# Ji4chenLi/t2v-turbo

Hardware: AMD Instinct MI355X
Metric: UNet denoise steps/sec (16f 320x512 latent) (higher is better)
Workload: dtype bf16; 1 GPU; VideoCrafter2 UNet forward, B=1 per GPU, latent (1,4,16,40,64), ctx (1,77,1024), 4-step LCM timestep table, random-init weights (zero-init tensors re-drawn); parallelism=replicas x1, hip_graph=True, graph_captured=True

## Files before the change

### include/t2v_hip.h

```cpp
#ifndef T2V_HIP_H
#define T2V_HIP_H

#ifdef __cplusplus
extern "C" {
#endif

#define T2V_OK 0
#define T2V_EINVAL (-1)
#define T2V_ESHAPE (-2)
#define T2V_EHIP (-3)

#define T2V_F32 0
#define T2V_BF16 1
#define T2V_F16 2

int t2v_version(void);
int t2v_init(void);
const char* t2v_last_error(void);

#define T2V_GEMM_LINEAR 0
#define T2V_GEMM_CONV3X3 1
#define T2V_GEMM_CONV3X3_S2 2
#define T2V_GEMM_CONV3X3_UP2 3
#define T2V_GEMM_TCONV3 4
// ... 103 lines not shown
                    float* ws, float* stats, void* stream);

int t2v_layernorm(const void* x, int ldx, int M, int C, const float* gamma, const float* beta,
                  float eps, void* out, int ldo, void* stream);

int t2v_softmax_rows(void* s, long long rows, int n, int n_pad, int ld, void* stream);

int t2v_attn_spatial(const void* q, int ldq, const void* k, int ldk, const void* vt, int ld_vt,
                     long long vt_img_stride, void* out, int ldo, int n_img, int seq_q, int seq_kv,
                     int heads, int kv_div, float scale, void* stream);

int t2v_attn_temporal(const void* q, int ldq, const void* k, int ldk, const void* v, int ldv,
                      void* out, int ldo, int n_clips, int frames, int hw, int heads, float scale,
                      float* probs, void* stream);

int t2v_ncfhw_to_tokens(const void* x, int dt, int b, int c, int f, int hw, void* out, int ldo,
                        void* stream);
int t2v_tokens_to_ncfhw(const void* tok, int tok_f32, int ld, int b, int c, int f, int hw,
                        void* out, int dt, void* stream);
int t2v_timestep_embedding(const void* t, int t_is_f32, int n, int dim, int guidance_style,
                           void* out_bf16, void* stream);
int t2v_silu(const void* x, void* out, long long n, void* stream);
int t2v_fill_zero(void* p, long long nbytes, void* stream);
int t2v_cast(const void* x, int dt_in, void* out, int dt_out, long long n, void* stream);
int t2v_lincomb3(const float* x, const float* y, const float* z, const float* ca, const float* cb,
                 const float* cc, int nb, long long inner, float* out, void* stream);
int t2v_lcm_step(const float* x, const void* eps, int eps_dt, const float* noise, float sa_t,
                 float sb_t, float c_skip, float c_out, float sa_p, float sb_p, long long n,
                 float* prev, float* denoised, void* stream);
int t2v_video_to_u8(const void* x, int dt, int B, int T, int H, int W, void* out, void* stream);
// ... 215 lines not shown
```

### t2v-turbo_amd/csrc/linear_pr.hip

```cpp
#include "gelu_poly.h"
#if defined(T2V_HOSTSIM) && !defined(T2V_WT_ON)
#define T2V_WT_ON(bit) 0
template <int WT, class V> inline void t2v_store_out16(void* p, const V& v) { *(V*)p = v; }
template <int WT, class V> inline void t2v_store_out8(void* p, const V& v) { *(V*)p = v; }
#endif
#include <cstdlib>
#include <type_traits>

struct LprParams {
    t2v_gemm_desc d;
    int chunks;
    int chunks_per_y;
    int n_out;
    int debug;
};

#ifdef T2V_LPR_ABLATE
#define LABL(bit) (p.debug & (bit))
#else
#define LABL(bit) false
#endif

#ifdef T2V_LPR_TRACE
#define LPR_STAMP() do { if (tr && ti < 31) { if (lane == 0) tr[ti] = __builtin_amdgcn_s_memtime(); ++ti; } } while (0)
#else
#define LPR_STAMP() do { } while (0)
#endif

namespace {
// ... 1 lines not shown
constexpr int kLprWaves = 8;
#ifndef T2V_LPR_RING
#define T2V_LPR_RING 5
#endif
#ifndef T2V_LPR_STAGGER
#define T2V_LPR_STAGGER 0
#endif
#ifdef T2V_LPR_PACKED_GELU
constexpr bool kLprScalarGelu = false;
#else
constexpr bool kLprScalarGelu = true;
#endif
#ifndef T2V_LPR_AF1
#define T2V_LPR_AF1 1
#endif
constexpr int kLprRing = T2V_LPR_RING;
constexpr bool kLprAf1 = T2V_LPR_AF1 != 0;

template <int I, int N, class F>
__device__ __forceinline__ void lpr_static_for(F&& f) {
    if constexpr (I < N) {
        f(std::integral_constant<int, I>{});
        lpr_static_for<I + 1, N>(f);
    }
}

template <int TB, int KS, int EPI, int PRE>
__global__ __launch_bounds__(kLprWaves * 64) __attribute__((amdgpu_waves_per_eu(2, 2))) void linear_pr_kernel(const LprParams p) {
    constexpr int BM = 32 * TB, K = 16 * KS, D = KS % kLprRing == 0 ? kLprRing : 4;
    constexpr bool GEGLU = EPI == 1, RES = EPI == 2;
    constexpr bool XPF = !RES;
// ... 19 lines not shown
    LPR_STAMP();
    unsigned long long* wg_tr = d.ws ? (unsigned long long*)d.ws + 3 * kLprWaves * 32 + (blockIdx.y * gridDim.x + blockIdx.x) * 4 : nullptr;
    if (wg_tr && tid == 0) { wg_tr[0] = __builtin_amdgcn_s_memtime(); wg_tr[2] = (unsigned)__builtin_amdgcn_s_getreg((15 << 11) | (0 << 6) | 4); wg_tr[3] = (unsigned)__builtin_amdgcn_s_getreg((3 << 11) | (0 << 6) | 20); }
#endif
    const int c_begin = blockIdx.y * p.chunks_per_y, c_end = min(p.chunks, c_begin + p.chunks_per_y);

    const int n_run = c_end - c_begin;
    const bool active = wave < n_run;
    int chunk = c_begin + (active ? wave : 0);

    uint4 rres[RES ? TB : 1][2][2];
    auto load_res_all = [&](int ch) {
        if constexpr (RES) {
            unsigned loff = (unsigned)lane;
            asm volatile("" : "+v"(loff));
            loff = ((loff & 31u) * (unsigned)d.ldr + 16u * (loff >> 5)) * 2u;
#pragma unroll
            for (int i = 0; i < TB; ++i) {
                const int row0 = m0 + 32 * i < d.M ? m0 + 32 * i : m0;
                const char* rp = (const char*)d.residual + ((long long)row0 * d.ldr + ch * 64) * 2 + loff;
#pragma unroll
                for (int b = 0; b < 2; ++b) {
                    rres[i][b][0] = *(const uint4*)(rp + 64 * b);
                    rres[i][b][1] = *(const uint4*)(rp + 64 * b + 16);
                }
            }
        }
    };

    constexpr bool LNIN = PRE == 1, GNIN = PRE == 2;
    if constexpr (PRE == 0) {
        constexpr int CG = K / 64, RG = BM / 8, PIECES = RG * CG, PPW = (PIECES + kLprWaves - 1) / kLprWaves;
        uint4 stage[PPW];
        const bf16_t* a = (const bf16_t*)d.a0;
#pragma unroll
// ... 2 lines not shown
            const int rg = pc / CG, cg = pc - rg * CG;
            const int row = 8 * rg + (lane & 7), c = 8 * cg + (lane >> 3);
            const int gm = m0 + row;
            if (pc < PIECES) stage[j] = *(const uint4*)(a + (long long)min(gm, d.M - 1) * d.lda0 + c * 8);
        }
        if (active) load_res_all(chunk);
        float* sb = (float*)(smem + PANEL_BYTES);
        const int nb = (c_end - c_begin) * 64;
        for (int i = tid; i < nb; i += kLprWaves * 64) sb[i] = d.bias ? d.bias[c_begin * 64 + i] : 0.f;
#pragma unroll
        for (int j = 0; j < PPW; ++j) {
            const int pc = wave + kLprWaves * j;
            const int rg = pc / CG, cg = pc - rg * CG;
            const int row = 8 * rg + (lane & 7), c = 8 * cg + (lane >> 3);
            if (pc < PIECES) *(uint4*)(smem + (c * BM + row) * 16) = m0 + row < d.M ? stage[j] : make_uint4(0u, 0u, 0u, 0u);
        }
    } else {
        constexpr int CG = K / 64, RG = BM / 8, RPW = (RG + kLprWaves - 1) / kLprWaves;
        uint4 stage[RPW][CG];
        const bf16_t* a = (const bf16_t*)d.a0;
#pragma unroll
        for (int jr = 0; jr < RPW; ++jr) {
            const int rg = wave + kLprWaves * jr;
            const int gm = m0 + 8 * rg + (lane & 7);
            const bf16_t* ap = a + (long long)min(gm, d.M - 1) * d.lda0 + (lane >> 3) * 8;
#pragma unroll
            for (int cg = 0; cg < CG; ++cg)
                if (rg < RG) stage[jr][cg] = *(const uint4*)(ap + cg * 64);
        }
        float* sb = (float*)(smem + PANEL_BYTES);
// ... 172 lines not shown
            const char* wb = wcur;
            static_assert(KS / D >= 2, "a first and a last iteration");
            lpr_static_for<0, D>([&](auto u) { kstep(wb, 0, u, F{}, T{}); });
            wb += D * 2048;
#pragma unroll 1
            for (int it = 1; it < KS / D - 1; ++it, wb += D * 2048) lpr_static_for<0, D>([&](auto u) { kstep(wb, it * D, u, F{}, F{}); });
            lpr_static_for<0, D>([&](auto u) { kstep(wb, KS - D, u, T{}, F{}); });
        }
        LPR_STAMP();
        int chunk_e = chunk;
        asm volatile("" : "+s"(chunk_e));
        {
            unsigned ao = a_off;
            asm volatile("" : "+v"(ao));
            const unsigned he = ao >= (unsigned)(BM * 16) ? 1u : 0u, le = (ao >> 4) - he * BM;
            const unsigned g_off = (le * (unsigned)d.ldo + 16u * he) * 2u;
            auto put = [&](const float* v, int row0, int col) {
                if (row0 + (int)le < d.M && !LABL(16)) {
                    char* op = (char*)obase + ((long long)row0 * d.ldo + col) * 2 + g_off;
                    t2v_store_out16<T2V_WT_ON(T2V_WT_LINEAR_PR)>(op, pack8(v));
                    t2v_store_out16<T2V_WT_ON(T2V_WT_LINEAR_PR)>(op + 16, pack8(v + 8));
                }
            };
            if constexpr (GEGLU) {
#pragma unroll
                for (int i = 0; i < TB; ++i) {
                    float v[16];
                    if (LABL(8)) {
#pragma unroll
                        for (int e = 0; e < 16; ++e) v[e] = acc[i][0][e] + acc[i][1][e];
                    } else if (LABL(64) || kLprScalarGelu) {
#pragma unroll
                        for (int e = 0; e < 16; ++e) v[e] = acc[i][0][e] * fast_gelu(acc[i][1][e]);
                    } else {
#pragma unroll
                        for (int e = 0; e < 16; e += 2) {
                            const f32x2_t gg = fast_gelu2((f32x2_t){acc[i][1][e], acc[i][1][e + 1]});
                            const f32x2_t vv = (f32x2_t){acc[i][0][e], acc[i][0][e + 1]} * gg;
                            v[e] = vv[0]; v[e + 1] = vv[1];
                        }
                    }
#ifdef T2V_LPR_TRACE
                    if (chunk < c_begin + kLprWaves) { asm volatile("" :: "v"(v[0]), "v"(v[15])); LPR_STAMP(); }
#endif
                    put(v, m0 + 32 * i, chunk_e * 32);
#ifdef T2V_LPR_TRACE
                    if (chunk < c_begin + kLprWaves) LPR_STAMP();
#endif
                }
            } else {
#pragma unroll
                for (int ib = 0; ib < 2 * TB; ++ib) {
                    const int i = ib >> 1, b = ib & 1;
                    float v[16];
#pragma unroll
                    for (int e = 0; e < 16; ++e) v[e] = acc[i][b][e];
                    put(v, m0 + 32 * i, chunk_e * 64 + 32 * b);
                }
            }
        }
        LPR_STAMP();
#ifdef T2V_LPR_TRACE
        if (!has_next && wg_tr && lane == 0) atomicMax(&wg_tr[1], (unsigned long long)__builtin_amdgcn_s_memtime());
#endif
        if (!has_next) break;
        chunk = nchunk;
        wcur = wnext;
        load_res_all(chunk);

    }
}

template <int TB, int KS, int EPI, int PRE = 0>
int lpr_launch(const LprParams& p, int tiles_m, int ny, hipStream_t s) {
    const int smem = 16 * KS * 32 * TB * 2 + p.chunks_per_y * 64 * 4;
    static bool attr_set = false;
    if (!attr_set) {
        hipFuncSetAttribute((const void*)linear_pr_kernel<TB, KS, EPI, PRE>, hipFuncAttributeMaxDynamicSharedMemorySize, 160 * 1024);
        attr_set = true;
    }
    hipLaunchKernelGGL((linear_pr_kernel<TB, KS, EPI, PRE>), dim3(tiles_m, ny), dim3(kLprWaves * 64), smem, s, p);
    T2V_CHECK_LAUNCH();
    return T2V_OK;
}

}

static int g_lpr_debug = 0, g_lpr_force_ny = 0;
extern "C" int t2v_linear_pr_debug(int bits) { g_lpr_debug = bits; return T2V_OK; }
extern "C" int t2v_linear_pr_force_split(int ny) { g_lpr_force_ny = ny; return T2V_OK; }

static int lpr_prepare(const t2v_gemm_desc* dd, LprParams& p, int& cfg, int& tiles_m, int& ny) {
    cfg = 0;
    T2V_REQUIRE(dd && dd->a0 && dd->w && dd->out, T2V_EINVAL, "t2v_linear_pr: null pointer");
    p.d = *dd;
    const t2v_gemm_desc& d = p.d;
    {
        const int n_out = d.act == T2V_ACT_GEGLU ? d.N / 2 : d.N;
        T2V_REQUIRE(d.lda0 >= d.c0 && (!d.a1 || d.lda1 >= d.c1), T2V_EINVAL, "t2v_linear_pr: lda0 < c0 or lda1 < c1");
        T2V_REQUIRE(d.ldo >= n_out && (!d.residual || d.ldr >= n_out) && (!d.rowvec || d.ld_rowvec >= n_out), T2V_EINVAL,
                    "t2v_linear_pr: ldo / ldr / ld_rowvec smaller than the output row");
    }
    if (d.mode != T2V_GEMM_LINEAR || d.a1 || d.c1 || d.batch > 1 || d.alpha != 1.0f || d.out_f32 || d.split_k > 1 || d.drop_thr || d.ln_out ||
        d.rowstat_out || d.colstat_out || d.lnf_stats || d.lora_t || d.rowvec || (d.act != T2V_ACT_NONE && d.act != T2V_ACT_GEGLU))
        return T2V_OK;
    if (d.c0 != 320 && d.c0 != 640 && d.c0 != 512) return T2V_OK;
    if (d.M <= 0 || d.N <= 0 || d.N % 64 || d.lda0 % 8 || d.ldo % 8) return T2V_OK;
    if ((long long)d.M * d.ldo >= (1ll << 31) || (long long)d.M * d.ldr >= (1ll << 31) || (long long)d.N * d.c0 * 2 >= (1ll << 31)) return T2V_OK;
    if (((uintptr_t)d.a0 | (uintptr_t)d.w | (uintptr_t)d.out) % 16) return T2V_OK;
    if (d.residual && (d.act == T2V_ACT_GEGLU || d.ldr % 8 || (uintptr_t)d.residual % 16 || d.M % 32)) return T2V_OK;
    if (d.bias && (uintptr_t)d.bias % 16) return T2V_OK;
    if (d.ln_in) {
        T2V_REQUIRE(d.ln_gamma && d.ln_beta, T2V_EINVAL, "t2v_linear_pr: ln_in without ln_gamma / ln_beta");
        if (d.residual || ((uintptr_t)d.ln_gamma | (uintptr_t)d.ln_beta) % 16) return T2V_OK;
    }
    const int bm = d.c0 == 320 ? 160 : 96;
    if (d.c0 == 512 && (d.residual || d.gn_coef)) return T2V_OK;
    if (d.gn_coef) {
        T2V_REQUIRE(!d.ln_in && d.gn_rows_per_unit > 0, T2V_EINVAL, "t2v_linear_pr: gn_coef with ln_in, or without gn_rows_per_unit");
        if (d.residual || (uintptr_t)d.gn_coef % 16 || d.gn_rows_per_unit % bm || d.M % d.gn_rows_per_unit) return T2V_OK;
    }
    p.chunks = d.N / 64;
    p.n_out = d.act == T2V_ACT_GEGLU ? d.N / 2 : d.N;
    tiles_m = (d.M + bm - 1) / bm;
    ny = 1;
    if (g_lpr_force_ny > 0) ny = g_lpr_force_ny;
    else if (tiles_m < 256) {
        ny = (256 + tiles_m / 2) / tiles_m;
        const int max_ny = p.chunks / kLprWaves > 0 ? p.chunks / kLprWaves : 1;
        if (ny > max_ny) ny = max_ny;
    }
    if (ny > p.chunks) ny = p.chunks;
    if (ny < 1) ny = 1;
    p.chunks_per_y = (p.chunks + ny - 1) / ny;
    ny = (p.chunks + p.chunks_per_y - 1) / p.chunks_per_y;
    if (d.c0 * bm * 2 + p.chunks_per_y * 256 > 160 * 1024) return T2V_OK;
    p.debug = g_lpr_debug;
    cfg = d.c0 == 320 ? 1 : (d.c0 == 640 ? 2 : 3);
    return T2V_OK;
}

extern "C" int t2v_linear_pr_supported(const t2v_gemm_desc* dd) {
    LprParams p;
    int cfg = 0, tiles_m = 0, ny = 0;
    const int rc = lpr_prepare(dd, p, cfg, tiles_m, ny);
    return rc != T2V_OK ? rc : (cfg > 0 ? 1 : 0);
}

extern "C" int t2v_linear_pr(const t2v_gemm_desc* dd, void* stream) {
    LprParams p;
    int cfg = 0, tiles_m = 0, ny = 0;
// ... 6 lines not shown
        T2V_REQUIRE(epi != 2 && !p.d.gn_coef, T2V_ESHAPE, "t2v_linear_pr: K = 512 takes the plain and the GEGLU epilogue (ask t2v_linear_pr_supported first)");
        if (p.d.ln_in) return epi == 1 ? lpr_launch<3, 32, 1, 1>(p, tiles_m, ny, s) : lpr_launch<3, 32, 0, 1>(p, tiles_m, ny, s);
        return epi == 1 ? lpr_launch<3, 32, 1>(p, tiles_m, ny, s) : lpr_launch<3, 32, 0>(p, tiles_m, ny, s);
    }
    if (p.d.ln_in) {
        if (cfg == 1) return epi == 1 ? lpr_launch<5, 20, 1, 1>(p, tiles_m, ny, s) : lpr_launch<5, 20, 0, 1>(p, tiles_m, ny, s);
        return epi == 1 ? lpr_launch<3, 40, 1, 1>(p, tiles_m, ny, s) : lpr_launch<3, 40, 0, 1>(p, tiles_m, ny, s);
    }
    if (p.d.gn_coef) {
        T2V_REQUIRE(epi == 0, T2V_ESHAPE, "t2v_linear_pr: gn_coef goes with the plain epilogue");
        return cfg == 1 ? lpr_launch<5, 20, 0, 2>(p, tiles_m, ny, s) : lpr_launch<3, 40, 0, 2>(p, tiles_m, ny, s);
    }
    if (cfg == 1) return epi == 1 ? lpr_launch<5, 20, 1>(p, tiles_m, ny, s) : (epi == 2 ? lpr_launch<5, 20, 2>(p, tiles_m, ny, s) : lpr_launch<5, 20, 0>(p, tiles_m, ny, s));
    return epi == 1 ? lpr_launch<3, 40, 1>(p, tiles_m, ny, s) : (epi == 2 ? lpr_launch<3, 40, 2>(p, tiles_m, ny, s) : lpr_launch<3, 40, 0>(p, tiles_m, ny, s));
}
```

### t2v-turbo_amd/csrc/replay.hip

```cpp
#include "common.h"

#include <cstring>
#include <tuple>
#include <type_traits>
#include <utility>

namespace {

template <class T>
inline T slot_as(uint64_t v) {
    if constexpr (std::is_pointer_v<T>) {
        return (T)(uintptr_t)v;
    } else if constexpr (std::is_same_v<T, float>) {
        const uint32_t b = (uint32_t)v;
        float f;
        memcpy(&f, &b, 4);
        return f;
    } else if constexpr (std::is_same_v<T, double>) {
        double d;
        memcpy(&d, &v, 8);
        return d;
    } else {
        return (T)(int64_t)v;
    }
// ... 23 lines not shown
const Entry kTable[] = {
    T2V_ENTRY(t2v_gemm), T2V_ENTRY(t2v_conv_halo), T2V_ENTRY(t2v_linear_pr),
#ifdef T2V_EXPERIMENTAL
    T2V_ENTRY(t2v_ffn_fused),
#endif
    T2V_ENTRY(t2v_conv3x3_small_cin), T2V_ENTRY(t2v_gn_stats),
    T2V_ENTRY(t2v_gn_apply), T2V_ENTRY(t2v_group_norm), T2V_ENTRY(t2v_group_norm_cs), T2V_ENTRY(t2v_gn_stats_cs), T2V_ENTRY(t2v_layernorm),
    T2V_ENTRY(t2v_softmax_rows), T2V_ENTRY(t2v_attn_spatial), T2V_ENTRY(t2v_attn_temporal), T2V_ENTRY(t2v_ncfhw_to_tokens),
    T2V_ENTRY(t2v_tokens_to_ncfhw), T2V_ENTRY(t2v_timestep_embedding), T2V_ENTRY(t2v_silu), T2V_ENTRY(t2v_fill_zero), T2V_ENTRY(t2v_cast),
    T2V_ENTRY(t2v_lincomb3), T2V_ENTRY(t2v_lcm_step), T2V_ENTRY(t2v_gn_bwd), T2V_ENTRY(t2v_softmax_bwd_rows), T2V_ENTRY(t2v_transpose_bf16),
    T2V_ENTRY(t2v_sumpool2x2), T2V_ENTRY(t2v_gn_bwd2), T2V_ENTRY(t2v_layernorm_bwd), T2V_ENTRY(t2v_geglu_fwd), T2V_ENTRY(t2v_geglu_bwd),
    T2V_ENTRY(t2v_scatter2x), T2V_ENTRY(t2v_add_bf16), T2V_ENTRY(t2v_attn_temporal_bwd), T2V_ENTRY(t2v_adamw_step), T2V_ENTRY(t2v_ema_update),
    T2V_ENTRY(t2v_sumsq), T2V_ENTRY(t2v_gather_f32), T2V_ENTRY(t2v_attn_spatial_bwd), T2V_ENTRY(t2v_wgrad_tn), T2V_ENTRY(t2v_wgrad_tn_group),
    T2V_ENTRY(t2v_transpose_pad_bf16), T2V_ENTRY(t2v_dropout_bf16), T2V_ENTRY(t2v_im2col_bf16), T2V_ENTRY(t2v_gn_coef_cs), T2V_ENTRY(t2v_norm_affine_grad),
    T2V_ENTRY(t2v_rowlin_fwd), T2V_ENTRY(t2v_rowlin_bwd_data), T2V_ENTRY(t2v_rowlin_wgrad), T2V_ENTRY(t2v_timestep_embedding_f32), T2V_ENTRY(t2v_dropout_f32),
    T2V_ENTRY(t2v_rank_loss), T2V_ENTRY(t2v_ema_multi),
};
constexpr int kEntries = (int)(sizeof(kTable) / sizeof(kTable[0]));

}

extern "C" int t2v_replay_lookup(const char* name) {
    if (!name) return -1;
    for (int i = 0; i < kEntries; ++i)
        if (strcmp(kTable[i].name, name) == 0) return i;
    return -1;
}


extern "C" int t2v_replay(const unsigned long long* prog, long long nwords, void* stream, int* failed_index) {
    T2V_REQUIRE(prog && nwords >= 0, T2V_EINVAL, "t2v_replay: null program");
// ... 18 lines not shown
```

### t2v-turbo_amd/engine.py

```python
import collections
import os

import torch
import torch.nn as nn

from . import native as nt
from .native import on_tensor_device
from .packs import Packer, effective_weight_bias, is_lora_leaf, leaf_out_channels, params_fingerprint, params_fingerprints
from .unet3d import (Downsample, ResBlock, SpatialTransformer, TemporalTransformer, TimestepEmbedSequential,
                     Upsample)


class BufferPool:

    def __init__(self, device):
        self.device = device
        self.free = collections.defaultdict(list)
        self.live = {}
        self.links = {}
        self.bytes = 0

    def get(self, rows, cols, dtype, zero=False):
        n = rows * cols
        nbytes = ((n * torch.empty((), dtype=dtype).element_size() + 255) // 256) * 256
# ... 158 lines not shown
    linear_pr = os.environ.get("T2V_LINEAR_PR", "1") == "1"
    linear_pr_min_n = {320: int(os.environ.get("T2V_LPR_MIN_N_320", "640")), 640: int(os.environ.get("T2V_LPR_MIN_N_640", "1920")),
                       512: int(os.environ.get("T2V_LPR_MIN_N_512", "1536"))}
    if os.environ.get("T2V_LPR_K512", "1") != "1":
        del linear_pr_min_n[512]

    def _lpr_takes(self, a, w, out, kw):
        if not self.linear_pr or any(k in kw for k in ("ln", "lnf", "colstat", "rowstat")) or not hasattr(self.ops, "linear_pr_supported"):
            return False
        K, N = a.shape[1], kw["N"]
        if K not in self.linear_pr_min_n or w.shape[1] != K or w.shape[0] != N or w.stride(0) != K:
            return False
        if kw.get("act") != nt.ACT_GEGLU and N < self.linear_pr_min_n[K]:
            return False
        return self.ops.linear_pr_supported(a, w, out, **kw) == 1

    ln_in_fill = os.environ.get("T2V_LN_IN", "1") == "1"

    def linear_ln_in(self, a, norm, *, w, bias, act=nt.ACT_NONE):
        if not self.ln_in_fill or tuple(norm.normalized_shape) != (a.shape[1],) or not norm.elementwise_affine:
            return None
        N = w.shape[0]
        out = self.buf(a.shape[0], N // 2 if act == nt.ACT_GEGLU else N)
        kw = dict(M=a.shape[0], N=N, bias=bias, residual=None, act=act,
                  ln_in=(self.pk.f32(norm.weight), self.pk.f32(norm.bias), norm.eps))
        if not self._lpr_takes(a, w, out, kw):
            self.pool.put(out)
            return None
        self.ops.linear_pr(a, self.pk.lpr(w), out, **kw)
        return out
# ... 553 lines not shown
            ops.layernorm(src, pk.f32(norm.weight), pk.f32(norm.bias), norm.eps, ln_buf())
            return box["ln"]

        def foldable(norm, stats):
            return (fold and stats is not None and tuple(norm.normalized_shape) == (C,) and norm.elementwise_affine and
                    C % 64 == 0 and C <= 1280)

        wide = fold and self.fold_ln_wide

        def folded(src, norm, stats, pack, act=nt.ACT_NONE):
            if not foldable(norm, stats):
                return None
            wp, s_vec, t_vec = pack()
            return self.linear(src, None, w=wp, bias=t_vec, act=act, lnf=(stats, norm.eps, s_vec))

        def temporal_attn(attn, norm, src, stats):
            qkv = folded(src, norm, stats if wide else None, lambda: pk.mat_lnf([attn.to_q, attn.to_k, attn.to_v], norm, "qkv_lnf"))
            if qkv is None and src is not box["ln"]:
                qkv = self.linear_ln_in(src, norm, w=pk.cat_mats([attn.to_q, attn.to_k, attn.to_v], "qkv"), bias=None)
            if qkv is None:
                qkv = self.linear(lnorm(norm, src) if src is not box["ln"] else src, None,
                                  w=pk.cat_mats([attn.to_q, attn.to_k, attn.to_v], "qkv"), bias=None)
            o = self.buf(M, inner)
            probs = None
            if attn.record_attn_probs:
                probs = torch.empty(B * hw * attn.heads, F, F, dtype=torch.float32, device=self.device)
                self.plan["probs"].append((attn, probs))
            ops.attn_temporal(qkv[:, :inner], qkv[:, inner:2 * inner], qkv[:, 2 * inner:], o, B, F, hw, attn.heads,
                              attn.scale, probs)
            self.pool.put(qkv)
            return o

        def spatial_self_attn(attn, src):
            qk = self.linear(src, None, w=pk.cat_mats([attn.to_q, attn.to_k], "qk"), bias=None)
            kp = ((hw + 63) // 64) * 64
            vt = self.buf(n_img * inner, kp)
            if kp != hw:
                ops.fill_zero(vt)
            ops.gemm(pk.mat(attn.to_v), src, vt, M=inner, N=hw, batch=n_img, w_strides=(hw * src.stride(0), 0),
                     o_strides=(inner * kp, 0))
            o = self.buf(M, inner)
            ops.attn_spatial(qk[:, :inner], qk[:, inner:], vt, kp, o, n_img, hw, hw, attn.heads, 1, attn.scale)
            self.pool.put(qk, vt)
            return o

        def cross_attn(attn, norm, src, stats):
            q = folded(src, norm, stats, lambda: pk.mat_lnf([attn.to_q], norm, "q_lnf"))
            if q is None:
                q = self.linear(lnorm(norm, src) if src is not box["ln"] else src, attn.to_q, bias=None)
            k, vt, kp, vt_stride = self.context_kv(attn)
            o = self.buf(M, inner)
            ops.attn_spatial(q, k, vt, kp, o, n_img, hw, self.ctx_len, attn.heads, F, attn.scale, vt_stride)
            self.pool.put(q)
            return o

        if temporal:
            o = temporal_attn(a1, blk.norm1, ln1 if ln1 is not None else y, rs)
        else:
            o = spatial_self_attn(a1, ln1 if ln1 is not None else lnorm(blk.norm1, y))
        y1 = self.linear(o, a1.to_out[0], residual=y, ln=(blk.norm2, ln_buf()) if fuse2 else None, want_rs=fold and (wide or not temporal))
        rs1 = self.last_rs
        self.pool.put(o)
        src = box["ln"] if fuse2 else y1
        o = temporal_attn(a2, blk.norm2, src, rs1) if temporal else cross_attn(a2, blk.norm2, src, rs1)
        y2 = self.linear(o, a2.to_out[0], residual=y1, ln=(blk.norm3, ln_buf()) if fuse3 else None, want_rs=wide)
        rs2 = self.last_rs
        self.pool.put(o, y1)
        proj = blk.ff.net[0]
        assert hasattr(proj, "proj"), "non-gated FeedForward is not built by the VideoCrafter2 config"
        if (self.fuse_ff and ops.ffn_fused_supported(C) and tuple(blk.norm3.normalized_shape) == (C,) and blk.norm3.elementwise_affine
                and not fuse3 and leaf_out_channels(blk.ff.net[2]) == C and leaf_out_channels(proj.proj) == 8 * C):
            w1p, b1p, w2p, b2f = pk.ffn(blk.ff, blk.norm3)
            y3 = self.buf(M, C)
            ops.ffn_fused(y2, w1p, b1p, w2p, b2f, blk.norm3.eps, y3)
            self.pool.put(y2, box["ln"])
            return y3
        g = folded(y2, blk.norm3, rs2 if wide else None, lambda: pk.geglu_lnf(proj.proj, blk.norm3), act=nt.ACT_GEGLU)
        if g is None and not fuse3:
            wg, bg = pk.geglu(proj.proj)
            g = self.linear_ln_in(y2, blk.norm3, w=wg, bias=bg, act=nt.ACT_GEGLU)
        if g is None:
            src = box["ln"] if fuse3 else lnorm(blk.norm3, y2)
# ... 69 lines not shown
```

### t2v-turbo_amd/native.py

```python
import ctypes as C
import os

import torch

_PKG = os.path.dirname(os.path.abspath(__file__))
LIB_PATH = os.path.join(_PKG, "libt2v_hip.so")

F32, BF16, F16 = 0, 1, 2
GEMM_LINEAR, GEMM_CONV3X3, GEMM_CONV3X3_S2, GEMM_CONV3X3_UP2, GEMM_TCONV3, GEMM_CONV3X3_S2_PAD01 = range(6)
ACT_NONE, ACT_GEGLU, ACT_SILU = 0, 1, 2

_DT = {torch.float32: F32, torch.bfloat16: BF16, torch.float16: F16}


WGRAD_GROUP_MAX = 8


class WgradProblem(C.Structure):
    _fields_ = [("a", C.c_void_p), ("b", C.c_void_p), ("out", C.c_void_p), ("M", C.c_longlong), ("lda", C.c_int), ("ldb", C.c_int),
                ("ldo", C.c_int), ("R", C.c_int), ("C", C.c_int), ("alpha", C.c_float)]


RANK_LOSS_MAX = 16
RANK_LOSS_WG_LANES = 2048
# ... 188 lines not shown
    "t2v_group_norm_cs_ws_floats": (C.c_longlong, [C.c_int, C.c_int, C.c_int]),
    "t2v_gn_stats_cs": (C.c_int, [C.c_void_p, C.c_int, C.c_void_p, C.c_int, C.c_int, C.c_int, C.c_int, C.c_float, C.c_void_p, C.c_void_p,
                                  C.c_void_p]),
    "t2v_group_norm_cs": (C.c_int, [C.c_void_p, C.c_void_p, C.c_void_p, C.c_int, C.c_int, C.c_void_p, C.c_int, C.c_int, C.c_int, C.c_int,
                                    C.c_int, C.c_float, C.c_void_p, C.c_void_p, C.c_int, C.c_void_p, C.c_void_p, C.c_int, C.c_void_p,
                                    C.c_longlong, C.c_void_p]),
    "t2v_layernorm": (C.c_int, [C.c_void_p, C.c_int, C.c_int, C.c_int, C.c_void_p, C.c_void_p, C.c_float,
                                C.c_void_p, C.c_int, C.c_void_p]),
    "t2v_softmax_rows": (C.c_int, [C.c_void_p, C.c_longlong, C.c_int, C.c_int, C.c_int, C.c_void_p]),
    "t2v_attn_spatial": (C.c_int, [C.c_void_p, C.c_int, C.c_void_p, C.c_int, C.c_void_p, C.c_int, C.c_longlong,
                                   C.c_void_p, C.c_int, C.c_int, C.c_int, C.c_int, C.c_int, C.c_int, C.c_float,
                                   C.c_void_p]),
    "t2v_attn_temporal": (C.c_int, [C.c_void_p, C.c_int, C.c_void_p, C.c_int, C.c_void_p, C.c_int, C.c_void_p,
                                    C.c_int, C.c_int, C.c_int, C.c_int, C.c_int, C.c_float, C.c_void_p,
                                    C.c_void_p]),
    "t2v_ncfhw_to_tokens": (C.c_int, [C.c_void_p, C.c_int, C.c_int, C.c_int, C.c_int, C.c_int, C.c_void_p, C.c_int,
                                      C.c_void_p]),
    "t2v_tokens_to_ncfhw": (C.c_int, [C.c_void_p, C.c_int, C.c_int, C.c_int, C.c_int, C.c_int, C.c_int, C.c_void_p,
                                      C.c_int, C.c_void_p]),
    "t2v_timestep_embedding": (C.c_int, [C.c_void_p, C.c_int, C.c_int, C.c_int, C.c_int, C.c_void_p, C.c_void_p]),
    "t2v_silu": (C.c_int, [C.c_void_p, C.c_void_p, C.c_longlong, C.c_void_p]),
    "t2v_fill_zero": (C.c_int, [C.c_void_p, C.c_longlong, C.c_void_p]),
    "t2v_cast": (C.c_int, [C.c_void_p, C.c_int, C.c_void_p, C.c_int, C.c_longlong, C.c_void_p]),
    "t2v_lincomb3": (C.c_int, [C.c_void_p, C.c_void_p, C.c_void_p, C.c_void_p, C.c_void_p, C.c_void_p, C.c_int,
                               C.c_longlong, C.c_void_p, C.c_void_p]),
    "t2v_gemm_debug": (C.c_int, [C.c_int]),
    "t2v_attn_debug": (C.c_int, [C.c_int]),
    "t2v_gn_coop_enable": (C.c_int, [C.c_int]),
    "t2v_gn_coop_error": (C.c_int, []),
    "t2v_gn_bwd_ws_floats": (C.c_longlong, [C.c_int, C.c_int, C.c_int]),
# ... 68 lines not shown
                                  C.c_float, C.c_void_p, C.c_void_p, C.c_void_p, C.c_longlong, C.c_void_p, C.c_int, C.c_longlong,
                                  C.c_void_p]),
    "t2v_cd_loss_bwd": (C.c_int, [C.c_void_p, C.c_void_p, C.c_void_p, C.c_void_p, C.c_void_p, C.c_int, C.c_int, C.c_longlong, C.c_void_p]),
    "t2v_cd_add_noise": (C.c_int, [C.c_void_p, C.c_void_p, C.c_int, C.c_void_p, C.c_int, C.c_void_p, C.c_void_p, C.c_int, C.c_int,
                                   C.c_longlong, C.c_void_p]),
    "t2v_ddim_reverse_step": (C.c_int, [C.c_void_p, C.c_int, C.c_int, C.c_void_p, C.c_void_p, C.c_int, C.c_void_p, C.c_void_p, C.c_int,
                                        C.c_int, C.c_longlong, C.c_void_p]),
    "t2v_pack_f16_multi": (C.c_int, [C.c_void_p, C.c_int, C.c_void_p, C.c_longlong, C.c_void_p]),
    "t2v_mp_guided_step": (C.c_int, [C.c_void_p, C.c_int, C.c_float, C.c_void_p, C.c_void_p, C.c_void_p, C.c_int, C.c_void_p, C.c_void_p,
                                     C.c_int, C.c_void_p, C.c_int, C.c_void_p, C.c_int, C.c_void_p, C.c_int, C.c_void_p, C.c_int,
                                     C.c_longlong, C.c_void_p]),
    "t2v_video_to_u8": (C.c_int, [C.c_void_p, C.c_int, C.c_int, C.c_int, C.c_int, C.c_int, C.c_void_p, C.c_void_p]),
}
EXPERIMENTAL = ("t2v_gemm2_enable", "t2v_ffn_fused_supported", "t2v_ffn_fused")
EXPORTED = sorted(n for n in _SIGS if n not in EXPERIMENTAL)


def has_experimental(lib=None):
    lib = lib if lib is not None else load()
    return hasattr(lib, "t2v_ffn_fused")


def load(path=None):
    global _lib
    if _lib is not None:
        return _lib
    path = path or os.environ.get("T2V_HIP_LIB", LIB_PATH)
    if not os.path.exists(path):
        raise NativeError(
            f"{path} not found: build it with `python __graft_entry__.py` / "
            f"`python t2v-turbo_amd/csrc/build.py` (hipcc, gfx950). There is no fallback path.")
    try:
        lib = C.CDLL(path)
    except OSError as e:
        raise NativeError(f"cannot load {path}: {e}") from e
    for name, (res, args) in _SIGS.items():
        if name in EXPERIMENTAL and not hasattr(lib, name):
            continue
        fn = getattr(lib, name)
        fn.restype = res
        fn.argtypes = args
    _lib = lib
    return lib


def _check(rc, what):
    if rc != 0:
        msg = _lib.t2v_last_error().decode(errors="replace") if _lib is not None else ""
        raise NativeError(f"{what} failed with code {rc}: {msg}")


def _p(t):
# ... 359 lines not shown
    def layernorm(self, x, gamma, beta, eps, out):
        self._call("t2v_layernorm", _p(x), _row_stride(x), x.shape[0], x.shape[1], _p(gamma), _p(beta), eps, _p(out),
                   _row_stride(out))

    def softmax_rows(self, s, rows, n, n_pad, ld):
        self._call("t2v_softmax_rows", _p(s), rows, n, n_pad, ld)

    def attn_spatial(self, q, k, vt, ld_vt, out, n_img, seq_q, seq_kv, heads, kv_div, scale, vt_img_stride=0):
        self._call("t2v_attn_spatial", _p(q), _row_stride(q), _p(k), _row_stride(k), _p(vt), ld_vt, vt_img_stride,
                   _p(out), _row_stride(out), n_img, seq_q, seq_kv, heads, kv_div, scale)

    def attn_temporal(self, q, k, v, out, n_clips, frames, hw, heads, scale, probs=None):
        self._call("t2v_attn_temporal", _p(q), _row_stride(q), _p(k), _row_stride(k), _p(v), _row_stride(v), _p(out),
                   _row_stride(out), n_clips, frames, hw, heads, scale, _p(probs))

    def ncfhw_to_tokens(self, x, out):
        b, c, f, h, w = x.shape
        assert x.is_contiguous()
        self._call("t2v_ncfhw_to_tokens", _p(x), _DT[x.dtype], b, c, f, h * w, _p(out), _row_stride(out))

    def tokens_to_ncfhw(self, tok, out):
        b, c, f, h, w = out.shape
        assert out.is_contiguous()
        self._call("t2v_tokens_to_ncfhw", _p(tok), 1 if tok.dtype == torch.float32 else 0, _row_stride(tok), b, c, f,
                   h * w, _p(out), _DT[out.dtype])

    def timestep_embedding(self, t, dim, guidance_style, out):
        assert t.dtype in (torch.int64, torch.float32) and t.is_contiguous()
        self._call("t2v_timestep_embedding", _p(t), 1 if t.dtype == torch.float32 else 0, t.numel(), dim,
                   int(guidance_style), _p(out))
# ... 335 lines not shown
```

Baseline: 47.42 steps/s.

## Fuse temporal attention into the to_out projection GEMM prologue

Adds a new PRE==3 prologue to the linear_pr kernel. The prologue computes 16-frame temporal attention per pixel and head with MFMA and writes the bf16 result straight into the GEMM's shared-memory A panel. The to_out projection with bias and residual then runs on that panel, so the attention output tensor no longer makes a round trip through global memory and one launch per temporal attention is removed. Tiles are remapped to clip/pixel panels with strided residual and output addressing. The fused path is limited to 320-wide blocks that are not fused or wide, and it adds extra LDS for the V transpose.

```diff
diff --git a/include/t2v_hip.h b/include/t2v_hip.h
--- a/include/t2v_hip.h
+++ b/include/t2v_hip.h
@@ -141,6 +141,11 @@
                       void* out, int ldo, int n_clips, int frames, int hw, int heads, float scale,
                       float* probs, void* stream);
 
+int t2v_attn_temporal_out(const void* q, int ldq, const void* k, int ldk, const void* v, int ldv,
+                          const t2v_gemm_desc* to_out, int n_clips, int frames, int hw, int heads, float scale, void* stream);
+int t2v_attn_temporal_out_supported(const void* q, int ldq, const void* k, int ldk, const void* v, int ldv,
+                                    const t2v_gemm_desc* to_out, int n_clips, int frames, int hw, int heads, float scale);
+
 int t2v_ncfhw_to_tokens(const void* x, int dt, int b, int c, int f, int hw, void* out, int ldo,
                         void* stream);
 int t2v_tokens_to_ncfhw(const void* tok, int tok_f32, int ld, int b, int c, int f, int hw,
diff --git a/t2v-turbo_amd/csrc/linear_pr.hip b/t2v-turbo_amd/csrc/linear_pr.hip
--- a/t2v-turbo_amd/csrc/linear_pr.hip
+++ b/t2v-turbo_amd/csrc/linear_pr.hip
@@ -6,6 +6,14 @@
 #endif
 #include <cstdlib>
 #include <type_traits>
+
+struct LprAttn {
+    const bf16_t *q, *k, *v;
+    int ldq, ldk, ldv;
+    int hw;
+    int panels_per_clip;
+    float c2;
+};
 
 struct LprParams {
     t2v_gemm_desc d;
@@ -13,6 +21,7 @@
     int chunks_per_y;
     int n_out;
     int debug;
+    LprAttn at;
 };
 
 #ifdef T2V_LPR_ABLATE
@@ -44,7 +53,14 @@
 #ifndef T2V_LPR_AF1
 #define T2V_LPR_AF1 1
 #endif
+#ifndef T2V_LPR_ATTN_AHEAD
+#define T2V_LPR_ATTN_AHEAD 1
+#endif
 constexpr int kLprRing = T2V_LPR_RING;
+constexpr int kLprAttnAhead = T2V_LPR_ATTN_AHEAD;
+constexpr int kLprVtLd = 20;
+constexpr int kLprVtBytes = 64 * kLprVtLd * 2;
+typedef __attribute__((__vector_size__(4 * sizeof(short)))) short lpr_bf16x4s_t;
 constexpr bool kLprAf1 = T2V_LPR_AF1 != 0;
 
 template <int I, int N, class F>
@@ -94,11 +110,20 @@
         if constexpr (RES) {
             unsigned loff = (unsigned)lane;
             asm volatile("" : "+v"(loff));
-            loff = ((loff & 31u) * (unsigned)d.ldr + 16u * (loff >> 5)) * 2u;
+            const unsigned hi = (loff >> 4) & 1u;
+            if constexpr (PRE == 3) loff = ((loff & 15u) * (unsigned)p.at.hw * (unsigned)d.ldr + 16u * (loff >> 5)) * 2u;
+            else loff = ((loff & 31u) * (unsigned)d.ldr + 16u * (loff >> 5)) * 2u;
 #pragma unroll
             for (int i = 0; i < TB; ++i) {
-                const int row0 = m0 + 32 * i < d.M ? m0 + 32 * i : m0;
-                const char* rp = (const char*)d.residual + ((long long)row0 * d.ldr + ch * 64) * 2 + loff;
+                const char* rp;
+                if constexpr (PRE == 3) {
+                    const int clip = blockIdx.x / p.at.panels_per_clip, p0 = (blockIdx.x - clip * p.at.panels_per_clip) * (BM / 16);
+                    const int px = min(2 * i + (int)hi, min(BM / 16, p.at.hw - p0) - 1);
+                    rp = (const char*)d.residual + (((long long)clip * 16 * p.at.hw + p0 + px) * d.ldr + ch * 64) * 2 + loff;
+                } else {
+                    const int row0 = m0 + 32 * i < d.M ? m0 + 32 * i : m0;
+                    rp = (const char*)d.residual + ((long long)row0 * d.ldr + ch * 64) * 2 + loff;
+                }
 #pragma unroll
                 for (int b = 0; b < 2; ++b) {
                     rres[i][b][0] = *(const uint4*)(rp + 64 * b);
@@ -131,6 +156,86 @@
             const int rg = pc / CG, cg = pc - rg * CG;
             const int row = 8 * rg + (lane & 7), c = 8 * cg + (lane >> 3);
             if (pc < PIECES) *(uint4*)(smem + (c * BM + row) * 16) = m0 + row < d.M ? stage[j] : make_uint4(0u, 0u, 0u, 0u);
+        }
+    } else if constexpr (PRE == 3) {
+        constexpr int P = BM / 16, HEADS = K / 64, ITEMS = P * HEADS, IPW = (ITEMS + kLprWaves - 1) / kLprWaves, PF = kLprAttnAhead;
+        const LprAttn& at = p.at;
+        const int clip = blockIdx.x / at.panels_per_clip, p0 = (blockIdx.x - clip * at.panels_per_clip) * P;
+        const int npix = min(P, at.hw - p0);
+        const int l15 = lane & 15, g = lane >> 4;
+        const long long row = ((long long)clip * 16 + l15) * at.hw + p0;
+        bf16_t* vt = (bf16_t*)(smem + PANEL_BYTES + p.chunks_per_y * 256 + wave * kLprVtBytes);
+        uint4 ld[PF + 1][6];
+        auto issue = [&](int j, int slot) {
+            const int it = wave + kLprWaves * j;
+            if (kLprWaves * (j + 1) <= ITEMS || it < ITEMS) {
+                const int pl = it / HEADS, head = it - pl * HEADS;
+                const long long r = row + min(pl, npix - 1);
+                const int col = head * 64 + g * 8;
+                const bf16_t *qp = at.q + r * at.ldq + col, *kp = at.k + r * at.ldk + col, *vp = at.v + r * at.ldv + col;
+                ld[slot][0] = *(const uint4*)qp; ld[slot][1] = *(const uint4*)(qp + 32);
+                ld[slot][2] = *(const uint4*)kp; ld[slot][3] = *(const uint4*)(kp + 32);
+                ld[slot][4] = *(const uint4*)vp; ld[slot][5] = *(const uint4*)(vp + 32);
+            }
+        };
+        auto item = [&](int j, int slot) {
+            const int it = wave + kLprWaves * j;
+            if (!(kLprWaves * (j + 1) <= ITEMS || it < ITEMS)) return;
+            const int pl = it / HEADS, head = it - pl * HEADS;
+            const f32x4_t zero4 = (f32x4_t){0.f, 0.f, 0.f, 0.f};
+            f32x4_t st = zero4;
+            st = __builtin_amdgcn_mfma_f32_16x16x32_bf16(*(bf16x8_t*)&ld[slot][2], *(bf16x8_t*)&ld[slot][0], st, 0, 0, 0);
+            st = __builtin_amdgcn_mfma_f32_16x16x32_bf16(*(bf16x8_t*)&ld[slot][3], *(bf16x8_t*)&ld[slot][1], st, 0, 0, 0);
+            __builtin_amdgcn_wave_barrier();
+            {
+                const uint4 v0 = ld[slot][4], v1 = ld[slot][5];
+                const uint32_t w[8] = {v0.x, v0.y, v0.z, v0.w, v1.x, v1.y, v1.z, v1.w};
+#pragma unroll
+                for (int e = 0; e < 8; ++e) {
+                    const int dd = g * 8 + (e >> 2) * 32 + (e & 3) * 2;
+                    vt[dd * kLprVtLd + l15] = (bf16_t)(w[e] & 0xffffu);
+                    vt[(dd + 1) * kLprVtLd + l15] = (bf16_t)(w[e] >> 16);
+                }
+            }
+            float sc[4];
+            float mloc = -INFINITY;
+#pragma unroll
+            for (int rr = 0; rr < 4; ++rr) { sc[rr] = st[rr]; mloc = fmaxf(mloc, sc[rr]); }
+            mloc = fmaxf(mloc, __shfl_xor(mloc, 16, 64));
+            mloc = fmaxf(mloc, __shfl_xor(mloc, 32, 64));
+            float lsum = 0.f;
+#pragma unroll
+            for (int rr = 0; rr < 4; ++rr) { sc[rr] = __builtin_amdgcn_exp2f((sc[rr] - mloc) * at.c2); lsum += sc[rr]; }
+            lsum += __shfl_xor(lsum, 16, 64);
+            lsum += __shfl_xor(lsum, 32, 64);
+            uint2 pu;
+            pu.x = pack2bf(sc[0], sc[1]);
+            pu.y = pack2bf(sc[2], sc[3]);
+            const lpr_bf16x4s_t pb = *(lpr_bf16x4s_t*)&pu;
+            __builtin_amdgcn_fence(__ATOMIC_RELEASE, "wavefront");
+            __builtin_amdgcn_wave_barrier();
+            const float inv = 1.f / lsum;
+            char* op = smem + (((head * 8 + (g >> 1)) * BM + 16 * pl + l15) * 16 + (g & 1) * 8);
+#pragma unroll
+            for (int m = 0; m < 4; ++m) {
+                const uint2 a = *(const uint2*)(vt + (m * 16 + l15) * kLprVtLd + 4 * g);
+                const f32x4_t o = __builtin_amdgcn_mfma_f32_16x16x16bf16_1k(*(const lpr_bf16x4s_t*)&a, pb, zero4, 0, 0, 0);
+                uint2 w;
+                w.x = pack2bf(o[0] * inv, o[1] * inv);
+                w.y = pack2bf(o[2] * inv, o[3] * inv);
+                *(uint2*)(op + m * (2 * BM * 16)) = pl < npix ? w : make_uint2(0u, 0u);
+            }
+        };
+#pragma unroll
+        for (int j = 0; j < PF && j < IPW; ++j) issue(j, j);
+        if (active) load_res_all(chunk);
+        float* sb = (float*)(smem + PANEL_BYTES);
+        const int nb = (c_end - c_begin) * 64;
+        for (int i = tid; i < nb; i += kLprWaves * 64) sb[i] = d.bias ? d.bias[c_begin * 64 + i] : 0.f;
+#pragma unroll
+        for (int j = 0; j < IPW; ++j) {
+            if (j + PF < IPW) issue(j + PF, (j + PF) % (PF + 1));
+            item(j, j % (PF + 1));
         }
     } else {
         constexpr int CG = K / 64, RG = BM / 8, RPW = (RG + kLprWaves - 1) / kLprWaves;
@@ -333,9 +438,19 @@
             unsigned ao = a_off;
             asm volatile("" : "+v"(ao));
             const unsigned he = ao >= (unsigned)(BM * 16) ? 1u : 0u, le = (ao >> 4) - he * BM;
-            const unsigned g_off = (le * (unsigned)d.ldo + 16u * he) * 2u;
-            auto put = [&](const float* v, int row0, int col) {
-                if (row0 + (int)le < d.M && !LABL(16)) {
+            const unsigned g_off = ((PRE == 3 ? (le & 15u) * (unsigned)p.at.hw + (le >> 4) : le) * (unsigned)d.ldo + 16u * he) * 2u;
+            auto put = [&](const float* v, int i, int col) {
+                int row0;
+                bool here;
+                if constexpr (PRE == 3) {
+                    const int clip = blockIdx.x / p.at.panels_per_clip, p0 = (blockIdx.x - clip * p.at.panels_per_clip) * (BM / 16);
+                    row0 = clip * 16 * p.at.hw + p0 + 2 * i;
+                    here = 2 * i + (int)(le >> 4) < min(BM / 16, p.at.hw - p0);
+                } else {
+                    row0 = m0 + 32 * i;
+                    here = row0 + (int)le < d.M;
+                }
+                if (here && !LABL(16)) {
                     char* op = (char*)obase + ((long long)row0 * d.ldo + col) * 2 + g_off;
                     t2v_store_out16<T2V_WT_ON(T2V_WT_LINEAR_PR)>(op, pack8(v));
                     t2v_store_out16<T2V_WT_ON(T2V_WT_LINEAR_PR)>(op + 16, pack8(v + 8));
@@ -362,7 +477,7 @@
 #ifdef T2V_LPR_TRACE
                     if (chunk < c_begin + kLprWaves) { asm volatile("" :: "v"(v[0]), "v"(v[15])); LPR_STAMP(); }
 #endif
-                    put(v, m0 + 32 * i, chunk_e * 32);
+                    put(v, i, chunk_e * 32);
 #ifdef T2V_LPR_TRACE
                     if (chunk < c_begin + kLprWaves) LPR_STAMP();
 #endif
@@ -374,7 +489,7 @@
                     float v[16];
 #pragma unroll
                     for (int e = 0; e < 16; ++e) v[e] = acc[i][b][e];
-                    put(v, m0 + 32 * i, chunk_e * 64 + 32 * b);
+                    put(v, i, chunk_e * 64 + 32 * b);
                 }
             }
         }
@@ -392,7 +507,7 @@
 
 template <int TB, int KS, int EPI, int PRE = 0>
 int lpr_launch(const LprParams& p, int tiles_m, int ny, hipStream_t s) {
-    const int smem = 16 * KS * 32 * TB * 2 + p.chunks_per_y * 64 * 4;
+    const int smem = 16 * KS * 32 * TB * 2 + p.chunks_per_y * 64 * 4 + (PRE == 3 ? kLprWaves * kLprVtBytes : 0);
     static bool attr_set = false;
     if (!attr_set) {
         hipFuncSetAttribute((const void*)linear_pr_kernel<TB, KS, EPI, PRE>, hipFuncAttributeMaxDynamicSharedMemorySize, 160 * 1024);
@@ -409,7 +524,7 @@
 extern "C" int t2v_linear_pr_debug(int bits) { g_lpr_debug = bits; return T2V_OK; }
 extern "C" int t2v_linear_pr_force_split(int ny) { g_lpr_force_ny = ny; return T2V_OK; }
 
-static int lpr_prepare(const t2v_gemm_desc* dd, LprParams& p, int& cfg, int& tiles_m, int& ny) {
+static int lpr_prepare(const t2v_gemm_desc* dd, LprParams& p, int& cfg, int& tiles_m, int& ny, int attn_hw = 0, int attn_clips = 0) {
     cfg = 0;
     T2V_REQUIRE(dd && dd->a0 && dd->w && dd->out, T2V_EINVAL, "t2v_linear_pr: null pointer");
     p.d = *dd;
@@ -427,21 +542,21 @@
     if (d.M <= 0 || d.N <= 0 || d.N % 64 || d.lda0 % 8 || d.ldo % 8) return T2V_OK;
     if ((long long)d.M * d.ldo >= (1ll << 31) || (long long)d.M * d.ldr >= (1ll << 31) || (long long)d.N * d.c0 * 2 >= (1ll << 31)) return T2V_OK;
     if (((uintptr_t)d.a0 | (uintptr_t)d.w | (uintptr_t)d.out) % 16) return T2V_OK;
-    if (d.residual && (d.act == T2V_ACT_GEGLU || d.ldr % 8 || (uintptr_t)d.residual % 16 || d.M % 32)) return T2V_OK;
+    if (d.residual && (d.act == T2V_ACT_GEGLU || d.ldr % 8 || (uintptr_t)d.residual % 16 || (d.M % 32 && !attn_hw))) return T2V_OK;
     if (d.bias && (uintptr_t)d.bias % 16) return T2V_OK;
     if (d.ln_in) {
         T2V_REQUIRE(d.ln_gamma && d.ln_beta, T2V_EINVAL, "t2v_linear_pr: ln_in without ln_gamma / ln_beta");
         if (d.residual || ((uintptr_t)d.ln_gamma | (uintptr_t)d.ln_beta) % 16) return T2V_OK;
     }
     const int bm = d.c0 == 320 ? 160 : 96;
-    if (d.c0 == 512 && (d.residual || d.gn_coef)) return T2V_OK;
+    if (d.c0 == 512 && ((d.residual && !attn_hw) || d.gn_coef)) return T2V_OK;
     if (d.gn_coef) {
         T2V_REQUIRE(!d.ln_in && d.gn_rows_per_unit > 0, T2V_EINVAL, "t2v_linear_pr: gn_coef with ln_in, or without gn_rows_per_unit");
         if (d.residual || (uintptr_t)d.gn_coef % 16 || d.gn_rows_per_unit % bm || d.M % d.gn_rows_per_unit) return T2V_OK;
     }
     p.chunks = d.N / 64;
     p.n_out = d.act == T2V_ACT_GEGLU ? d.N / 2 : d.N;
-    tiles_m = (d.M + bm - 1) / bm;
+    tiles_m = attn_hw ? attn_clips * ((attn_hw + bm / 16 - 1) / (bm / 16)) : (d.M + bm - 1) / bm;
     ny = 1;
     if (g_lpr_force_ny > 0) ny = g_lpr_force_ny;
     else if (tiles_m < 256) {
@@ -453,7 +568,7 @@
     if (ny < 1) ny = 1;
     p.chunks_per_y = (p.chunks + ny - 1) / ny;
     ny = (p.chunks + p.chunks_per_y - 1) / p.chunks_per_y;
-    if (d.c0 * bm * 2 + p.chunks_per_y * 256 > 160 * 1024) return T2V_OK;
+    if (d.c0 * bm * 2 + p.chunks_per_y * 256 + (attn_hw ? kLprWaves * kLprVtBytes : 0) > 160 * 1024) return T2V_OK;
     p.debug = g_lpr_debug;
     cfg = d.c0 == 320 ? 1 : (d.c0 == 640 ? 2 : 3);
     return T2V_OK;
@@ -490,3 +605,52 @@
     if (cfg == 1) return epi == 1 ? lpr_launch<5, 20, 1>(p, tiles_m, ny, s) : (epi == 2 ? lpr_launch<5, 20, 2>(p, tiles_m, ny, s) : lpr_launch<5, 20, 0>(p, tiles_m, ny, s));
     return epi == 1 ? lpr_launch<3, 40, 1>(p, tiles_m, ny, s) : (epi == 2 ? lpr_launch<3, 40, 2>(p, tiles_m, ny, s) : lpr_launch<3, 40, 0>(p, tiles_m, ny, s));
 }
+
+static int lpr_attn_prepare(const void* q, int ldq, const void* k, int ldk, const void* v, int ldv, const t2v_gemm_desc* to_out, int n_clips,
+                            int frames, int hw, int heads, float scale, LprParams& p, int& cfg, int& tiles_m) {
+    cfg = 0;
+    T2V_REQUIRE(q && k && v && to_out, T2V_EINVAL, "t2v_attn_temporal_out: null pointer");
+    T2V_REQUIRE(n_clips > 0 && frames > 0 && hw > 0 && heads > 0, T2V_EINVAL, "t2v_attn_temporal_out: bad size");
+    T2V_REQUIRE(ldq % 8 == 0 && ldk % 8 == 0 && ldv % 8 == 0, T2V_ESHAPE, "t2v_attn_temporal_out: strides");
+    T2V_REQUIRE(ldq >= heads * 64 && ldk >= heads * 64 && ldv >= heads * 64, T2V_ESHAPE, "t2v_attn_temporal_out: row stride smaller than heads * 64");
+    const long long M = (long long)n_clips * frames * hw;
+    if (frames != 16 || heads * 64 != to_out->c0 || !(scale > 0.f) || M >= (1ll << 31)) return T2V_OK;
+    if (M * ldq >= (1ll << 31) || M * ldk >= (1ll << 31) || M * ldv >= (1ll << 31)) return T2V_OK;
+    if (((uintptr_t)q | (uintptr_t)k | (uintptr_t)v) % 16) return T2V_OK;
+    t2v_gemm_desc dd = *to_out;
+    dd.a0 = q;
+    dd.lda0 = ldq;
+    if (dd.M != (int)M || !dd.residual || dd.act != T2V_ACT_NONE || dd.ln_in || dd.gn_coef) return T2V_OK;
+    int ny = 0;
+    const int rc = lpr_prepare(&dd, p, cfg, tiles_m, ny, hw, n_clips);
+    if (rc != T2V_OK) return rc;
+    if (ny != 1) cfg = 0;
+    if (!cfg) return T2V_OK;
+    const int pixels = cfg == 1 ? 10 : 6;
+    p.at.q = (const bf16_t*)q; p.at.k = (const bf16_t*)k; p.at.v = (const bf16_t*)v;
+    p.at.ldq = ldq; p.at.ldk = ldk; p.at.ldv = ldv;
+    p.at.hw = hw;
+    p.at.panels_per_clip = (hw + pixels - 1) / pixels;
+    p.at.c2 = scale * 1.4426950408889634f;
+    return T2V_OK;
+}
+
+extern "C" int t2v_attn_temporal_out_supported(const void* q, int ldq, const void* k, int ldk, const void* v, int ldv, const t2v_gemm_desc* to_out,
+                                               int n_clips, int frames, int hw, int heads, float scale) {
+    LprParams p;
+    int cfg = 0, tiles_m = 0;
+    const int rc = lpr_attn_prepare(q, ldq, k, ldk, v, ldv, to_out, n_clips, frames, hw, heads, scale, p, cfg, tiles_m);
+    return rc != T2V_OK ? rc : (cfg > 0 ? 1 : 0);
+}
+
+extern "C" int t2v_attn_temporal_out(const void* q, int ldq, const void* k, int ldk, const void* v, int ldv, const t2v_gemm_desc* to_out, int n_clips,
+                                     int frames, int hw, int heads, float scale, void* stream) {
+    LprParams p;
+    int cfg = 0, tiles_m = 0;
+    const int rc = lpr_attn_prepare(q, ldq, k, ldk, v, ldv, to_out, n_clips, frames, hw, heads, scale, p, cfg, tiles_m);
+    if (rc != T2V_OK) return rc;
+    T2V_REQUIRE(cfg > 0, T2V_ESHAPE, "t2v_attn_temporal_out: this launch is not taken (ask t2v_attn_temporal_out_supported first)");
+    hipStream_t s = (hipStream_t)stream;
+    if (cfg == 3) return lpr_launch<3, 32, 2, 3>(p, tiles_m, 1, s);
+    return cfg == 1 ? lpr_launch<5, 20, 2, 3>(p, tiles_m, 1, s) : lpr_launch<3, 40, 2, 3>(p, tiles_m, 1, s);
+}
diff --git a/t2v-turbo_amd/csrc/replay.hip b/t2v-turbo_amd/csrc/replay.hip
--- a/t2v-turbo_amd/csrc/replay.hip
+++ b/t2v-turbo_amd/csrc/replay.hip
@@ -61,7 +61,7 @@
     T2V_ENTRY(t2v_sumsq), T2V_ENTRY(t2v_gather_f32), T2V_ENTRY(t2v_attn_spatial_bwd), T2V_ENTRY(t2v_wgrad_tn), T2V_ENTRY(t2v_wgrad_tn_group),
     T2V_ENTRY(t2v_transpose_pad_bf16), T2V_ENTRY(t2v_dropout_bf16), T2V_ENTRY(t2v_im2col_bf16), T2V_ENTRY(t2v_gn_coef_cs), T2V_ENTRY(t2v_norm_affine_grad),
     T2V_ENTRY(t2v_rowlin_fwd), T2V_ENTRY(t2v_rowlin_bwd_data), T2V_ENTRY(t2v_rowlin_wgrad), T2V_ENTRY(t2v_timestep_embedding_f32), T2V_ENTRY(t2v_dropout_f32),
-    T2V_ENTRY(t2v_rank_loss), T2V_ENTRY(t2v_ema_multi),
+    T2V_ENTRY(t2v_rank_loss), T2V_ENTRY(t2v_ema_multi), T2V_ENTRY(t2v_attn_temporal_out),
 };
 constexpr int kEntries = (int)(sizeof(kTable) / sizeof(kTable[0]));
 
diff --git a/t2v-turbo_amd/engine.py b/t2v-turbo_amd/engine.py
--- a/t2v-turbo_amd/engine.py
+++ b/t2v-turbo_amd/engine.py
@@ -196,6 +196,28 @@
         if kw.get("act") != nt.ACT_GEGLU and N < self.linear_pr_min_n[K]:
             return False
         return self.ops.linear_pr_supported(a, w, out, **kw) == 1
+
+    attn_to_out = os.environ.get("T2V_ATTN_TO_OUT", "1") == "1"
+    attn_to_out_widths = tuple(int(c) for c in os.environ.get("T2V_ATTN_TO_OUT_WIDTHS", "320").split(",") if c)
+
+    def attn_temporal_to_out(self, attn, qkv, residual, hw):
+        ops, inner = self.ops, attn.heads * attn.dim_head
+        if (not self.linear_pr or not self.attn_to_out or not self.fold_ln or not hasattr(ops, "attn_temporal_out_supported")
+                or inner not in self.attn_to_out_widths or attn.record_attn_probs):
+            return None
+        mod = attn.to_out[0]
+        w, bias = self.pk.mat(mod), self.pk.bias(mod)
+        if w.shape[1] != inner or w.stride(0) != inner:
+            return None
+        out = self.buf(qkv.shape[0], w.shape[0])
+        args = (qkv[:, :inner], qkv[:, inner:2 * inner], qkv[:, 2 * inner:])
+        geom = (self.B, self.F, hw, attn.heads, attn.scale)
+        if ops.attn_temporal_out_supported(*args, w, out, *geom, bias=bias, residual=residual) != 1:
+            self.pool.put(out)
+            return None
+        ops.attn_temporal_out(*args, self.pk.lpr(w), out, *geom, bias=bias, residual=residual)
+        self.last_cs = self.last_rs = None
+        return out
 
     ln_in_fill = os.environ.get("T2V_LN_IN", "1") == "1"
 
@@ -779,13 +801,18 @@
             wp, s_vec, t_vec = pack()
             return self.linear(src, None, w=wp, bias=t_vec, act=act, lnf=(stats, norm.eps, s_vec))
 
-        def temporal_attn(attn, norm, src, stats):
+        def temporal_attn(attn, norm, src, stats, to_out_residual=None):
             qkv = folded(src, norm, stats if wide else None, lambda: pk.mat_lnf([attn.to_q, attn.to_k, attn.to_v], norm, "qkv_lnf"))
             if qkv is None and src is not box["ln"]:
                 qkv = self.linear_ln_in(src, norm, w=pk.cat_mats([attn.to_q, attn.to_k, attn.to_v], "qkv"), bias=None)
             if qkv is None:
                 qkv = self.linear(lnorm(norm, src) if src is not box["ln"] else src, None,
                                   w=pk.cat_mats([attn.to_q, attn.to_k, attn.to_v], "qkv"), bias=None)
+            if to_out_residual is not None:
+                y_out = self.attn_temporal_to_out(attn, qkv, to_out_residual, hw)
+                if y_out is not None:
+                    self.pool.put(qkv)
+                    return None, y_out
             o = self.buf(M, inner)
             probs = None
             if attn.record_attn_probs:
@@ -794,7 +821,7 @@
             ops.attn_temporal(qkv[:, :inner], qkv[:, inner:2 * inner], qkv[:, 2 * inner:], o, B, F, hw, attn.heads,
                               attn.scale, probs)
             self.pool.put(qkv)
-            return o
+            return o, None
 
         def spatial_self_attn(attn, src):
             qk = self.linear(src, None, w=pk.cat_mats([attn.to_q, attn.to_k], "qk"), bias=None)
@@ -819,18 +846,26 @@
             self.pool.put(q)
             return o
 
+        y1 = None
         if temporal:
-            o = temporal_attn(a1, blk.norm1, ln1 if ln1 is not None else y, rs)
+            o, y1 = temporal_attn(a1, blk.norm1, ln1 if ln1 is not None else y, rs, to_out_residual=None if fuse2 or wide else y)
         else:
             o = spatial_self_attn(a1, ln1 if ln1 is not None else lnorm(blk.norm1, y))
-        y1 = self.linear(o, a1.to_out[0], residual=y, ln=(blk.norm2, ln_buf()) if fuse2 else None, want_rs=fold and (wide or not temporal))
+        if y1 is None:
+            y1 = self.linear(o, a1.to_out[0], residual=y, ln=(blk.norm2, ln_buf()) if fuse2 else None, want_rs=fold and (wide or not temporal))
+            self.pool.put(o)
         rs1 = self.last_rs
-        self.pool.put(o)
         src = box["ln"] if fuse2 else y1
-        o = temporal_attn(a2, blk.norm2, src, rs1) if temporal else cross_attn(a2, blk.norm2, src, rs1)
-        y2 = self.linear(o, a2.to_out[0], residual=y1, ln=(blk.norm3, ln_buf()) if fuse3 else None, want_rs=wide)
+        y2 = None
+        if temporal:
+            o, y2 = temporal_attn(a2, blk.norm2, src, rs1, to_out_residual=None if fuse3 or wide else y1)
+        else:
+            o = cross_attn(a2, blk.norm2, src, rs1)
+        if y2 is None:
+            y2 = self.linear(o, a2.to_out[0], residual=y1, ln=(blk.norm3, ln_buf()) if fuse3 else None, want_rs=wide)
+            self.pool.put(o)
         rs2 = self.last_rs
-        self.pool.put(o, y1)
+        self.pool.put(y1)
         proj = blk.ff.net[0]
         assert hasattr(proj, "proj"), "non-gated FeedForward is not built by the VideoCrafter2 config"
         if (self.fuse_ff and ops.ffn_fused_supported(C) and tuple(blk.norm3.normalized_shape) == (C,) and blk.norm3.elementwise_affine
diff --git a/t2v-turbo_amd/native.py b/t2v-turbo_amd/native.py
--- a/t2v-turbo_amd/native.py
+++ b/t2v-turbo_amd/native.py
@@ -226,6 +226,10 @@
     "t2v_attn_temporal": (C.c_int, [C.c_void_p, C.c_int, C.c_void_p, C.c_int, C.c_void_p, C.c_int, C.c_void_p,
                                     C.c_int, C.c_int, C.c_int, C.c_int, C.c_int, C.c_float, C.c_void_p,
                                     C.c_void_p]),
+    "t2v_attn_temporal_out": (C.c_int, [C.c_void_p, C.c_int, C.c_void_p, C.c_int, C.c_void_p, C.c_int, C.POINTER(GemmDesc),
+                                        C.c_int, C.c_int, C.c_int, C.c_int, C.c_float, C.c_void_p]),
+    "t2v_attn_temporal_out_supported": (C.c_int, [C.c_void_p, C.c_int, C.c_void_p, C.c_int, C.c_void_p, C.c_int, C.POINTER(GemmDesc),
+                                                  C.c_int, C.c_int, C.c_int, C.c_int, C.c_float]),
     "t2v_ncfhw_to_tokens": (C.c_int, [C.c_void_p, C.c_int, C.c_int, C.c_int, C.c_int, C.c_int, C.c_void_p, C.c_int,
                                       C.c_void_p]),
     "t2v_tokens_to_ncfhw": (C.c_int, [C.c_void_p, C.c_int, C.c_int, C.c_int, C.c_int, C.c_int, C.c_int, C.c_void_p,
@@ -324,6 +328,7 @@
 }
 EXPERIMENTAL = ("t2v_gemm2_enable", "t2v_ffn_fused_supported", "t2v_ffn_fused")
 EXPORTED = sorted(n for n in _SIGS if n not in EXPERIMENTAL)
+OPTIONAL = ("t2v_attn_temporal_out", "t2v_attn_temporal_out_supported")
 
 
 def has_experimental(lib=None):
@@ -345,7 +350,7 @@
     except OSError as e:
         raise NativeError(f"cannot load {path}: {e}") from e
     for name, (res, args) in _SIGS.items():
-        if name in EXPERIMENTAL and not hasattr(lib, name):
+        if name in EXPERIMENTAL + OPTIONAL and not hasattr(lib, name):
             continue
         fn = getattr(lib, name)
         fn.restype = res
@@ -735,6 +740,21 @@
         self._call("t2v_attn_temporal", _p(q), _row_stride(q), _p(k), _row_stride(k), _p(v), _row_stride(v), _p(out),
                    _row_stride(out), n_clips, frames, hw, heads, scale, _p(probs))
 
+    def _attn_out_args(self, q, k, v, wp, out, n_clips, frames, hw, heads, scale, bias, residual):
+        d = self._gemm_desc(q, wp, out, M=out.shape[0], N=wp.shape[0], bias=bias, residual=residual, tile_cfg=-1)
+        return (_p(q), _row_stride(q), _p(k), _row_stride(k), _p(v), _row_stride(v), C.byref(d), n_clips, frames, hw, heads, scale)
+
+    def attn_temporal_out(self, q, k, v, wp, out, n_clips, frames, hw, heads, scale, *, bias=None, residual=None):
+        self._call("t2v_attn_temporal_out", *self._attn_out_args(q, k, v, wp, out, n_clips, frames, hw, heads, scale, bias, residual))
+
+    def attn_temporal_out_supported(self, q, k, v, wp, out, n_clips, frames, hw, heads, scale, *, bias=None, residual=None):
+        if not hasattr(self.lib, "t2v_attn_temporal_out_supported"):
+            return 0
+        rc = self.lib.t2v_attn_temporal_out_supported(*self._attn_out_args(q, k, v, wp, out, n_clips, frames, hw, heads, scale, bias, residual))
+        if rc < 0:
+            _check(rc, "t2v_attn_temporal_out_supported")
+        return rc
+
     def ncfhw_to_tokens(self, x, out):
         b, c, f, h, w = x.shape
         assert x.is_contiguous()
```

After: 47.73 steps/s (median of 6 runs). No clear change (+0.6%).
